# philip-bl/dctn

Measured on AMD Instinct MI355X. Metric: EPS-contraction windows/sec (fwd+bwd), higher is better.
Workload: dtype bf16; 1 GPU; cfg2 EPS[(3,4)]+linear bf16 B1024/GPU; parallelism=dp1

## Files before the change

### dctn_amd/csrc/common.h

```cpp
#pragma once
#include <hip/hip_runtime.h>
#include <stdint.h>

#include "../../include/dctn_amd.h"

typedef __bf16 bf16_t;

template <typename S> struct AccOf { typedef float type; };
template <> struct AccOf<double> { typedef double type; };

#define DCTN_WAVE 64

#ifndef DCTN_WT_FEATURES
#define DCTN_WT_FEATURES 16
#endif
#ifndef DCTN_WT_TILES
#define DCTN_WT_TILES 0
#endif

struct DctnDev { int cus; int lds; };
const DctnDev& dctn_dev();
int dctn_lds_wg_max();
long long dctn_resident_wgs(size_t lds_bytes, int lo, int hi);
bool dctn_lds_optin(const void* fn, size_t bytes);

#define DCTN_CHECK_LAUNCH()                                   \
  do {                                                        \
    if (hipGetLastError() != hipSuccess) return DCTN_ERR_LAUNCH; \
  } while (0)

void dctn_set_last_kernel(const char* name);

int dctn_zero_async(void* ptr, size_t bytes, hipStream_t st);

static inline long long ipow_ll(long long b, int e) {
  long long r = 1;
  for (int i = 0; i < e; ++i) r *= b;
  return r;
}

static inline size_t dtype_size(int dtype) {
  return dtype == DCTN_F64 ? 8 : (dtype == DCTN_F32 ? 4 : 2);
}

template <typename T>
__device__ __forceinline__ T wave_reduce_sum(T v) {
#pragma unroll
  for (int off = 32; off > 0; off >>= 1) v += __shfl_xor(v, off, 64);
  return v;
}

__device__ __forceinline__ void philox4x32_10(unsigned c0, unsigned c1, unsigned c2, unsigned c3, unsigned k0,
                                              unsigned k1, unsigned (&w)[4]) {
#pragma unroll
  for (int r = 0; r < 10; ++r) {
    const unsigned hi0 = __umulhi(0xD2511F53u, c0), lo0 = 0xD2511F53u * c0;
    const unsigned hi1 = __umulhi(0xCD9E8D57u, c2), lo1 = 0xCD9E8D57u * c2;
    c0 = hi1 ^ c1 ^ k0, c1 = lo1, c2 = hi0 ^ c3 ^ k1, c3 = lo0;
    k0 += 0x9E3779B9u, k1 += 0xBB67AE85u;
  }
  w[0] = c0, w[1] = c1, w[2] = c2, w[3] = c3;
}

struct EpsP {
  int C, B, H, W, Q, K, O, N, Ho, Wo;
  long long Wn;
  long long R;
  long long s[5];
  int m, LO, NH;
  long long HI;
  int bits;
  int opts;
};

int eps_fill_params(EpsP& p, const int64_t x_strides[5], int C, int B, int H, int W, int Q, int K,
                    int O, int policy = 0);

int eps_fwd_generic(const void* x, const void* core, void* out, void* ws, size_t ws_bytes, EpsP p, int dtype,
                    hipStream_t st);
size_t eps_bwd_generic_workspace(const EpsP& p, int dtype, int need_dx, int need_dcore);
int eps_bwd_generic(const void* x, const void* core, const void* dY, void* dX, void* dCore,
                    void* ws, size_t ws_bytes, EpsP p, int dtype, hipStream_t st);

int eps_gather_dx_launch(const void* gxw, void* dX, const EpsP& p, int dtype, hipStream_t st);

size_t eps_fwd_bigcore_workspace(const EpsP& p, int dtype, int precision);
size_t eps_bigcore_saved_bytes(const EpsP& p, int dtype, int precision);
int eps_fwd_bigcore(const void* x, const void* core, void* out, void* ws, size_t ws_bytes,
                    const EpsP& p, int dtype, int precision, hipStream_t st, void* zsave = nullptr);
size_t eps_bwd_dcore_bigcore_workspace(const EpsP& p, int dtype, int precision);
int eps_bwd_dcore_bigcore(const void* x, const void* dY, void* dCore, const EpsP& p, int dtype,
                          int precision, hipStream_t st, void* ws = nullptr, size_t ws_bytes = 0);
size_t eps_bwd_dfactor_bigcore_workspace(const EpsP& p, int dtype, int precision);
int eps_bwd_dx_bigcore(const void* x, const void* core, const void* dY, void* dX, void* ws,
                       size_t ws_bytes, const EpsP& p, int dtype, int precision, hipStream_t st,
                       const void* zsaved = nullptr, size_t zsaved_bytes = 0);

bool eps_bf16x3_covers(const EpsP& p, int dtype, int precision);
size_t eps_fwd_bf16x3_workspace(const EpsP& p, int dtype, int precision);
size_t eps_bf16x3_saved_bytes(const EpsP& p, int dtype, int precision);
int eps_fwd_bf16x3(const void* x, const void* core, void* out, void* ws, size_t ws_bytes, const EpsP& p, int dtype,
                   int precision, hipStream_t st, void* zsave = nullptr);
size_t eps_bwd_dfactor_bf16x3_workspace(const EpsP& p, int dtype, int precision);
int eps_bwd_dx_bf16x3(const void* x, const void* core, const void* dY, void* dX, void* ws, size_t ws_bytes, const EpsP& p,
                      int dtype, int precision, hipStream_t st, const void* zsaved = nullptr, size_t zsaved_bytes = 0);
size_t eps_bwd_dcore_bf16x3_workspace(const EpsP& p, int dtype, int precision);
int eps_bwd_dcore_bf16x3(const void* x, const void* dY, void* dCore, const EpsP& p, int dtype, int precision,
                         hipStream_t st, void* ws = nullptr, size_t ws_bytes = 0);

bool eps_q2f32_covers(const EpsP& p, int dtype, int precision);
int eps_fwd_q2f32(const void* x, const void* core, void* out, const EpsP& p, int dtype, int precision, hipStream_t st);
size_t eps_bwd_q2f32_workspace(const EpsP& p, int dtype, int precision);
int eps_bwd_q2f32(const void* x, const void* dY, void* dCore, void* ws, size_t ws_bytes, const EpsP& p, int dtype,
                  int precision, hipStream_t st);
int eps_head_fwd_q2f32(const void* x, const void* core, const void* head_w, const void* bias, void* feat, void* logits,
                       const EpsP& p, int Cout, int dtype, int precision, hipStream_t st);
size_t eps_head_bwd_q2f32_workspace(const EpsP& p, int Cout, int dtype, int precision);
int eps_head_bwd_q2f32(const void* x, const void* feat, const void* dLogits, const void* head_w, void* dCore, void* dW,
                       void* dBias, void* ws, size_t ws_bytes, const EpsP& p, int Cout, int dtype, int precision,
                       hipStream_t st);

bool eps_mfma_covers(const EpsP& p, int dtype, int precision);
bool eps_bigcore_covers(const EpsP& p, int dtype, int precision);

bool eps_halves_wanted(const EpsP& p, int dtype);
size_t eps_fwd_halves_workspace(const EpsP& p, int dtype);
size_t eps_halves_saved_bytes(const EpsP& p, int dtype);
int eps_fwd_halves(const void* x, const void* core, void* out, void* ws, size_t ws_bytes, const EpsP& p, int dtype,
                   hipStream_t st, void* saved = nullptr);
size_t eps_bwd_halves_workspace(const EpsP& p, int dtype, int need_dx, int need_dcore);
int eps_bwd_halves(const void* x, const void* core, const void* dY, void* dX, void* dCore, void* ws, size_t ws_bytes,
                   const EpsP& p, int dtype, hipStream_t st, const void* saved = nullptr, size_t saved_bytes = 0);

int eps_fwd_mfma(const void* x, const void* core, void* out, const EpsP& p, int dtype,
                 int precision, hipStream_t st, double* stats = nullptr);
int eps_out_stats(const void* y, long long n, int dtype, double* stats, hipStream_t st);
size_t eps_bwd_mfma_workspace(const EpsP& p, int dtype, int precision, int need_dx, int need_dcore);
int eps_bwd_mfma(const void* x, const void* core, const void* dY, void* dX, void* dCore, void* ws,
                 size_t ws_bytes, const EpsP& p, int dtype, int precision, hipStream_t st);
int eps_head_fwd_mfma(const void* x, const void* core, const void* head_w, const void* bias, void* feat, void* logits,
                      const EpsP& p, int Cout, int dtype, int precision, hipStream_t st);
size_t eps_head_bwd_mfma_workspace(const EpsP& p, int Cout, int dtype, int precision);
int eps_head_bwd_mfma(const void* x, const void* feat, const void* dLogits, const void* head_w, void* dCore,
                      void* dW, void* dBias, void* ws, size_t ws_bytes, const EpsP& p, int Cout, int dtype,
                      int precision, hipStream_t st);

struct SbsShape {
  int n;
  const int *out_sizes, *bond_sizes, *pos_h, *pos_w;
  int C, B, H, W, q, dtype;
};
static inline SbsShape sbs_string(SbsShape many, int i) {
  many.out_sizes += i * many.n;
  many.bond_sizes += i * many.n;
  many.pos_h += i * many.n;
  many.pos_w += i * many.n;
  return many;
}

size_t convsbs_saved_states_bytes(const SbsShape& sh);
int convsbs_fwd_mfma(const void* x, const int64_t xs[5], const void* const* cores, void* out, const SbsShape& sh,
                     hipStream_t st, float* save_states = nullptr);
int convsbs_bwd_mfma(const void* x, const int64_t xs[5], const void* const* cores, const void* dY, float* states, float* gxw,
                     float* const* dcores, const SbsShape& sh, hipStream_t st, float* partials = nullptr,
                     size_t partial_bytes = 0, const float* saved_states = nullptr);
bool convsbs_band_covers(const SbsShape& sh);
size_t convsbs_band_bwd_workspace(const SbsShape& sh);
int convsbs_fwd_band(const void* x, const int64_t xs[5], const void* const* cores, void* out, const SbsShape& sh,
                     hipStream_t st);
int convsbs_bwd_band(const void* x, const int64_t xs[5], const void* const* cores, const void* dY, void* dX,
// ... 22 lines not shown
```

### dctn_amd/csrc/eps_mfma.hip

```cpp
#include "common.h"

#include <cstdlib>
#include <type_traits>

typedef __attribute__((ext_vector_type(8))) __bf16 bf16x8;
typedef __attribute__((ext_vector_type(16))) float f32x16;
typedef __attribute__((ext_vector_type(8))) float f32x8;
typedef __attribute__((ext_vector_type(2))) int int2v;
typedef __attribute__((ext_vector_type(4))) int int4v;
typedef __attribute__((ext_vector_type(2))) float f32x2;

namespace {

constexpr int ilog2(int v) { return v <= 1 ? 0 : 1 + ilog2(v >> 1); }

template <typename S> __device__ __forceinline__ float to_f32(S v) { return (float)v; }

__device__ __forceinline__ float half_sum(float v) {
  const int iv = __float_as_int(v);
  const int2v r = __builtin_amdgcn_permlane32_swap(iv, iv, false, false);
  return __int_as_float(r[0]) + __int_as_float(r[1]);
}

__device__ __forceinline__ void swap_halves(float& a, float& b) {
  const int2v r = __builtin_amdgcn_permlane32_swap(__float_as_int(a), __float_as_int(b), false, false);
  a = __int_as_float(r[0]);
  b = __int_as_float(r[1]);
}
__device__ __forceinline__ void swap_halves(bf16x8& a, bf16x8& b) {
  int4v ia = __builtin_bit_cast(int4v, a), ib = __builtin_bit_cast(int4v, b);
#pragma unroll
  for (int i = 0; i < 4; ++i) {
    const int2v r = __builtin_amdgcn_permlane32_swap(ia[i], ib[i], false, false);
    ia[i] = r[0];
    ib[i] = r[1];
  }
  a = __builtin_bit_cast(bf16x8, ia);
  b = __builtin_bit_cast(bf16x8, ib);
}

__device__ __forceinline__ void wave_lds_sync() {
  __builtin_amdgcn_fence(__ATOMIC_RELEASE, "wavefront");
  __builtin_amdgcn_wave_barrier();
  __builtin_amdgcn_fence(__ATOMIC_ACQUIRE, "wavefront");
}

typedef short s16x4 __attribute__((ext_vector_type(4)));
typedef short s16x8 __attribute__((ext_vector_type(8)));
constexpr int LROW = 32;
struct TrLane {
  int wr[4];
  int rd_lo, rd_hi;
};
__device__ __forceinline__ TrLane tr_lane(int lane) {
  TrLane t;
#pragma unroll
  for (int c = 0; c < 4; ++c) t.wr[c] = lane * LROW + (((c + (lane >> 1)) & 3) << 3);
  const int g = lane >> 4, q = (lane >> 2) & 3, pp = lane & 3;
  const int lc = 2 * (g & 1) + (pp >> 1), half = pp & 1;
  const int row = 8 * (g >> 1) + q;
  t.rd_lo = row * LROW + (((lc + (row >> 1)) & 3) << 3) + 4 * half;
  t.rd_hi = (row + 4) * LROW + (((lc + ((row + 4) >> 1)) & 3) << 3) + 4 * half;
  return t;
}
__device__ __forceinline__ bf16x8 tr_frag(const short* tile, int ks, const TrLane& t) {
  typedef __attribute__((address_space(3))) s16x4 lds_s16x4;
  const s16x4 lo = __builtin_amdgcn_ds_read_tr16_b64_v4i16((lds_s16x4*)(tile + t.rd_lo + ks * 16 * LROW));
  const s16x4 hi = __builtin_amdgcn_ds_read_tr16_b64_v4i16((lds_s16x4*)(tile + t.rd_hi + ks * 16 * LROW));
  const s16x8 v = {lo[0], lo[1], lo[2], lo[3], hi[0], hi[1], hi[2], hi[3]};
  return __builtin_bit_cast(bf16x8, v);
}

struct FastDiv {
  unsigned M, s1, s2;
};
__device__ __forceinline__ unsigned fdiv(unsigned n, const FastDiv& d) {
  const unsigned t = __umulhi(d.M, n);
  return (t + ((n - t) >> d.s1)) >> d.s2;
}

#define MFMA_MAXN 16
struct MfmaP {
  int C, B, K, O, Ho, Wo;
  int P;
  int npg;
  int spc, nchunks;
  unsigned foffb[MFMA_MAXN];
  unsigned rowoffb[MFMA_MAXN];
  unsigned s1b, s2b, s3b, s4b;
  unsigned x_bytes;
  unsigned o_bytes, o_s1b;
  FastDiv div_wo;
  int rowvec_ok;
  int vec_ok;
  int Cout;
  unsigned hw_rowb, hw_bytes;
  int ncb;
  int skew;
  int opts;
#ifdef DCTN_STAMPS
  unsigned long long* stamps;
#endif
};

#ifdef DCTN_STAMPS
#define DCTN_STAMP(P, SLOT)                                                                      \
  do {                                                                                           \
    __builtin_amdgcn_sched_barrier(0);                                                           \
    unsigned long long t_;                                                                       \
    asm volatile("s_memrealtime %0\n\ts_waitcnt lgkmcnt(0)" : "=s"(t_)::"memory");               \
    if ((P).stamps && threadIdx.x == 0) (P).stamps[(long long)blockIdx.x * 8 + (SLOT)] = t_;     \
    __builtin_amdgcn_sched_barrier(0);                                                           \
  } while (0)
static unsigned long long* g_stamps = nullptr;
void dctn_stamps_set(unsigned long long* p) { g_stamps = p; }
__device__ unsigned long long* g_dev_stamps = nullptr;
void dctn_reduce_stamps_set(unsigned long long* p) { (void)hipMemcpyToSymbol(HIP_SYMBOL(g_dev_stamps), &p, sizeof(p)); }
#define DCTN_STAMP_T(P, SLOT, TID)                                                              \
  do {                                                                                           \
    __builtin_amdgcn_sched_barrier(0);                                                           \
    unsigned long long t_;                                                                       \
    asm volatile("s_memrealtime %0\n\ts_waitcnt lgkmcnt(0)" : "=s"(t_)::"memory");               \
    if ((P).stamps && threadIdx.x == (TID)) (P).stamps[(long long)blockIdx.x * 8 + (SLOT)] = t_;  \
    __builtin_amdgcn_sched_barrier(0);                                                           \
  } while (0)
#define DCTN_STAMP_ROLE_ROW 1024
#define DCTN_STAMP_R(P, SLOT)                                                                    \
  do {                                                                                           \
    __builtin_amdgcn_sched_barrier(0);                                                           \
    unsigned long long t_;                                                                       \
    asm volatile("s_memrealtime %0\n\ts_waitcnt lgkmcnt(0)" : "=s"(t_)::"memory");               \
    if ((P).stamps && threadIdx.x == 64 * 8)                                                     \
      (P).stamps[(long long)(DCTN_STAMP_ROLE_ROW + blockIdx.x) * 8 + (SLOT)] = t_;               \
    __builtin_amdgcn_sched_barrier(0);                                                           \
  } while (0)
#define DCTN_STAMP_WAVE_ROW 1536
#define DCTN_STAMP_W(P, WV)                                                                      \
  do {                                                                                           \
    __builtin_amdgcn_sched_barrier(0);                                                           \
    unsigned long long t_;                                                                       \
    asm volatile("s_memrealtime %0\n\ts_waitcnt lgkmcnt(0)" : "=s"(t_)::"memory");               \
    if ((P).stamps && (threadIdx.x & 63) == 0 && (WV) < 8)                                        \
      (P).stamps[(long long)(DCTN_STAMP_WAVE_ROW + blockIdx.x) * 8 + (WV)] = t_;                 \
    __builtin_amdgcn_sched_barrier(0);                                                           \
  } while (0)
#define DCTN_STAMP_G(SLOT)                                                                       \
  do {                                                                                           \
    __builtin_amdgcn_sched_barrier(0);                                                           \
    unsigned long long t_;                                                                       \
    asm volatile("s_memrealtime %0\n\ts_waitcnt lgkmcnt(0)" : "=s"(t_)::"memory");               \
    if (g_dev_stamps && threadIdx.x == 0) g_dev_stamps[(long long)blockIdx.x * 8 + (SLOT)] = t_;  \
    __builtin_amdgcn_sched_barrier(0);                                                           \
  } while (0)
#else
#define DCTN_STAMP(P, SLOT) do { } while (0)
#define DCTN_STAMP_T(P, SLOT, TID) do { } while (0)
#define DCTN_STAMP_G(SLOT) do { } while (0)
#define DCTN_STAMP_R(P, SLOT) do { } while (0)
#define DCTN_STAMP_W(P, WV) do { } while (0)
#endif

typedef __attribute__((ext_vector_type(4))) unsigned u32x4;
typedef __attribute__((ext_vector_type(2))) unsigned u32x2;
typedef __attribute__((ext_vector_type(2))) __bf16 bf16x2;

__device__ __forceinline__ __amdgpu_buffer_rsrc_t make_rsrc(const void* ptr, unsigned bytes) {
  return __builtin_amdgcn_make_buffer_rsrc(const_cast<void*>(ptr), 0, (int)bytes, 0x00020000);
}

template <typename S, int N, bool VEC, int ROWS>
struct RawWindow {
  u32x4 row[ROWS > 0 ? ROWS : 1];
  unsigned v[(ROWS == 0 && VEC) ? N * (int)(sizeof(S) / 2) : 1];
  unsigned e[(ROWS == 0 && !VEC) ? 2 * N : 1];
};

template <typename S, int N, bool VEC, int ROWS>
__device__ __forceinline__ void issue_window(__amdgpu_buffer_rsrc_t rs, unsigned voff, unsigned soff,
                                             const MfmaP& p, RawWindow<S, N, VEC, ROWS>& raw) {
  if constexpr (ROWS > 0) {
#pragma unroll
    for (int rw = 0; rw < ROWS; ++rw)
      raw.row[rw] = __builtin_amdgcn_raw_buffer_load_b128(rs, voff, soff + p.rowoffb[rw], 0);
  } else if constexpr (VEC) {
#pragma unroll
    for (int n = 0; n < N; ++n) {
      if constexpr (sizeof(S) == 2) {
        raw.v[n] = __builtin_amdgcn_raw_buffer_load_b32(rs, voff, soff + p.foffb[n], 0);
      } else {
        const u32x2 t = __builtin_amdgcn_raw_buffer_load_b64(rs, voff, soff + p.foffb[n], 0);
        raw.v[2 * n] = t.x;
        raw.v[2 * n + 1] = t.y;
      }
    }
  } else {
#pragma unroll
    for (int n = 0; n < N; ++n)
#pragma unroll
      for (int q = 0; q < 2; ++q) {
        if constexpr (sizeof(S) == 2)
          raw.e[2 * n + q] = (unsigned)(unsigned short)__builtin_amdgcn_raw_buffer_load_b16(
              rs, voff, soff + p.foffb[n] + q * p.s4b, 0);
        else
          raw.e[2 * n + q] = __builtin_amdgcn_raw_buffer_load_b32(rs, voff, soff + p.foffb[n] + q * p.s4b, 0);
      }
  }
}

template <typename S, int N, bool VEC, int ROWS>
__device__ __forceinline__ void unpack_window(const RawWindow<S, N, VEC, ROWS>& raw, float (&xv)[N][2]) {
  if constexpr (ROWS > 0) {
    constexpr int KK = N / ROWS;
    constexpr int CC = ROWS * ROWS / N;
#pragma unroll
    for (int rw = 0; rw < ROWS; ++rw) {
      const unsigned d[4] = {raw.row[rw].x, raw.row[rw].y, raw.row[rw].z, raw.row[rw].w};
#pragma unroll
      for (int dw = 0; dw < KK; ++dw) {
        const int n = ((rw / CC) * KK + dw) * CC + (rw % CC);
        xv[n][0] = __uint_as_float(d[dw] << 16);
        xv[n][1] = __uint_as_float(d[dw] & 0xffff0000u);
      }
    }
  } else if constexpr (VEC) {
#pragma unroll
    for (int n = 0; n < N; ++n) {
      if constexpr (sizeof(S) == 2) {
        xv[n][0] = __uint_as_float(raw.v[n] << 16);
        xv[n][1] = __uint_as_float(raw.v[n] & 0xffff0000u);
      } else {
        xv[n][0] = __uint_as_float(raw.v[2 * n]);
        xv[n][1] = __uint_as_float(raw.v[2 * n + 1]);
      }
    }
  } else {
#pragma unroll
    for (int n = 0; n < N; ++n)
#pragma unroll
      for (int q = 0; q < 2; ++q)
        xv[n][q] = sizeof(S) == 2 ? __uint_as_float(raw.e[2 * n + q] << 16) : __uint_as_float(raw.e[2 * n + q]);
  }
}

template <typename S, int OP>
struct RawRow {
  static constexpr int DW = OP * (int)sizeof(S) / 4;
  unsigned d[DW];
  unsigned e[OP];
};
template <typename S, int OP, bool VEC>
__device__ __forceinline__ void issue_row(__amdgpu_buffer_rsrc_t rs, unsigned voff, unsigned soff, int O,
                                          RawRow<S, OP>& r) {
// ... 334 lines not shown
    }
    core_commit(e0, tmp);
  }
  __syncthreads();
  bf16x8 cf[MT][KS];
#pragma unroll
  for (int t = 0; t < MT; ++t)
#pragma unroll
    for (int s = 0; s < KS; ++s)
      cf[t][s] = *reinterpret_cast<const bf16x8*>(&cs[((t * KS + s) * 64 + lane) * 8]);
#pragma unroll
  for (int u = 1; u < HEAD_FWD_HS; ++u)
    issue_window<S, N, true, ROWS>(rs_x, voff_x, (unsigned)first_of_group(u) * p.s1b, p, raw[u]);
  bf16x8 wf[HK];
  {
    const __amdgpu_buffer_rsrc_t rs_hw = make_rsrc(hw, p.hw_bytes);
    const int c = lane & 15, g = lane >> 4;
    const unsigned base = c < p.Cout ? (unsigned)c * p.hw_rowb + (unsigned)(wv * 64 * OP + 8 * g) * 2u : p.hw_bytes;
#pragma unroll
    for (int ks = 0; ks < HK; ++ks)
      wf[ks] = __builtin_bit_cast(bf16x8, __builtin_amdgcn_raw_buffer_load_b128(rs_hw, base, (unsigned)(ks * 64), 0));
  }
  __builtin_amdgcn_sched_barrier(0);

  short* tile = &ftile[wv][0];
  const int bcol = (lane & 15) < HEAD_FWD_HS ? (lane & 15) : HEAD_FWD_HS - 1;
  const short* brd = tile + bcol * SROW + 8 * (lane >> 4);
  DCTN_STAMP(p, 1);
  for (int g0 = b0, grp = 0; g0 < b1; g0 += HEAD_FWD_HS, ++grp) {
    const int g1 = g0 + HEAD_FWD_HS < b1 ? g0 + HEAD_FWD_HS : b1;
#pragma unroll
    for (int u = 0; u < HEAD_FWD_HS; ++u) {
      const int b = g0 + u;
      if (b >= g1) break;
      float xv[N][2];
      unpack_window<S, N, true, ROWS>(raw[u], xv);
      {
        const int bn = b + HEAD_FWD_HS < b1 ? b + HEAD_FWD_HS : b1 - 1;
        issue_window<S, N, true, ROWS>(rs_x, voff_x, (unsigned)bn * p.s1b, p, raw[u]);
        __builtin_amdgcn_sched_barrier(0);
      }
      bf16x8 pf0[KS], pf1[KS];
      build_p0<N0>(xv, pf0, pf1);
#pragma unroll
      for (int s = 0; s < KS; ++s) swap_halves(pf0[s], pf1[s]);
      float m0[BN / 2], m1[BN / 2];
      {
        float ph[BN / 2];
        ph[0] = xv[N - 2][0];
        ph[1] = xv[N - 2][1];
#pragma unroll
        for (int u = 2; u < N1; ++u)
#pragma unroll
          for (int bh = (1 << (u - 1)) - 1; bh >= 0; --bh) {
            const f32x2 pr = bmul2(ph[bh], f32x2{xv[N - 1 - u][0], xv[N - 1 - u][1]});
            ph[bh] = pr[0];
            ph[bh | (1 << (u - 1))] = pr[1];
          }
#pragma unroll
        for (int bh = 0; bh < BN / 2; ++bh) {
          const f32x2 mm = bmul2(ph[bh], f32x2{xv[N - 1][0], xv[N - 1][1]});
          m0[bh] = mm[0];
          m1[bh] = mm[1];
          swap_halves(m0[bh], m1[bh]);
        }
      }
      float res0[OP], res1[OP];
#pragma unroll
      for (int o = 0; o < OP; ++o) { res0[o] = 0.f; res1[o] = 0.f; }
#pragma unroll
      for (int t = 0; t < MT; ++t) {
#pragma unroll
        for (int set = 0; set < 2; ++set) {
          f32x16 acc;
#pragma unroll
          for (int v = 0; v < 16; ++v) acc[v] = 0.f;
#pragma unroll
          for (int s = 0; s < KS; ++s)
            acc = __builtin_amdgcn_mfma_f32_32x32x16_bf16(cf[t][s], set ? pf1[s] : pf0[s], acc, 0, 0, 0);
#pragma unroll
          for (int v = 0; v < 16; v += 2) {
            const int code = (t << 4) | ((v >> 2) << 2) | (v & 3);
            const float mm = set ? m1[code >> LOGO] : m0[code >> LOGO];
            float* dst = set ? res1 : res0;
            const int o = code & (OP - 1);
            const f32x2 r = bfma2(mm, f32x2{acc[v], acc[v + 1]}, f32x2{dst[o], dst[o + 1]});
            dst[o] = r[0];
            dst[o + 1] = r[1];
          }
        }
      }
      unsigned pk[OP / 2];
#pragma unroll
      for (int i = 0; i < OP / 2; ++i) {
        float a0 = res0[2 * i], a1 = res1[2 * i], c0 = res0[2 * i + 1], c1 = res1[2 * i + 1];
        swap_halves(a0, a1);
        swap_halves(c0, c1);
        pk[i] = pack_bf16(a0 + a1, c0 + c1);
      }
      if constexpr (OP == 2) {
        __builtin_amdgcn_raw_buffer_store_b32(pk[0], rs_o, voff_o, (unsigned)b * p.o_s1b, 0);
        *reinterpret_cast<unsigned*>(tile + (b - g0) * SROW + lane * OP) = pk[0];
      } else if constexpr (OP == 4) {
        __builtin_amdgcn_raw_buffer_store_b64(u32x2{pk[0], pk[1]}, rs_o, voff_o, (unsigned)b * p.o_s1b, 0);
        *reinterpret_cast<u32x2*>(tile + (b - g0) * SROW + lane * OP) = u32x2{pk[0], pk[1]};
      } else {
#pragma unroll
        for (int i = 0; i < OP / 8; ++i) {
          const u32x4 q = u32x4{pk[4 * i], pk[4 * i + 1], pk[4 * i + 2], pk[4 * i + 3]};
          __builtin_amdgcn_raw_buffer_store_b128(q, rs_o, voff_o, (unsigned)b * p.o_s1b + 16u * i, 0);
          *reinterpret_cast<u32x4*>(tile + (b - g0) * SROW + lane * OP + 8 * i) = q;
        }
      }
      if (b == b0) DCTN_STAMP(p, 2);
    }
    wave_lds_sync();
    f32x4v hd = {0.f, 0.f, 0.f, 0.f};
#pragma unroll
    for (int ks = 0; ks < HK; ++ks) {
      const bf16x8 fb = *reinterpret_cast<const bf16x8*>(brd + 32 * ks);
      hd = __builtin_amdgcn_mfma_f32_16x16x32_bf16(wf[ks], fb, hd, 0, 0, 0);
    }
    wave_lds_sync();
    {
      const int sl = lane & 15, cb = 4 * (lane >> 4);
      if (sl < g1 - g0) {
#pragma unroll
        for (int v = 0; v < 4; ++v) hsum[grp & 1][sl][cb + v][wv] = hd[v];
      }
    }
    DCTN_STAMP(p, 3);
    __syncthreads();
    for (int e = tid; e < (g1 - g0) * p.Cout; e += (int)blockDim.x) {
      const int sl = e / p.Cout, c = e - sl * p.Cout;
      float t = (float)bias[c];
      for (int w = 0; w < nwv; ++w) t += hsum[grp & 1][sl][c][w];
      logits[(long long)(g0 + sl) * p.Cout + c] = (bf16_t)t;
    }
  }
  DCTN_STAMP(p, 4);
}

constexpr int HEADT_WAVES = 16;
constexpr int HEADT_GS = 4;
constexpr int HEADT_MAXKS = 6;
constexpr int headt_pitch(int F) { return (F + 31) / 32 * 32 + 8; }

template <int N0, int N1, int OP, int ROWS, bool BLK4>
__global__ __launch_bounds__(64 * HEADT_WAVES) void eps_fwd_head_q2reg_t_k(const bf16_t* __restrict__ x,
                                                                           const bf16_t* __restrict__ core,
                                                                           const bf16_t* __restrict__ hw,
                                                                           const bf16_t* __restrict__ bias,
                                                                           bf16_t* __restrict__ out,
                                                                           bf16_t* __restrict__ logits, MfmaP p) {
  typedef bf16_t S;
  typedef __attribute__((ext_vector_type(4))) float f32x4v;
  constexpr int N = N0 + N1, A = 1 << N0, BN = 1 << N1, KS = A / 16, MT = BN * OP / 32;
  constexpr int LOGO = ilog2(OP);
  constexpr int TOT = A * BN * OP;
  static_assert(OP % 2 == 0 && TOT % 4 == 0, "outputs are handled as bf16 pairs");
  __shared__ __attribute__((aligned(16))) bf16_t cs[TOT];
  __shared__ float hsum[HEADT_WAVES][HEADT_GS][16];
  __shared__ unsigned step_ctr;
  extern __shared__ __attribute__((aligned(16))) short ftile[];
  const int tid = threadIdx.x, lane = tid & 63;
  const int wv = __builtin_amdgcn_readfirstlane(tid >> 6);
  const int b0 = (int)blockIdx.x * p.spc, b1 = b0 + p.spc < p.B ? b0 + p.spc : p.B;
  const int F = p.P * OP, LP = headt_pitch(F);
  const __amdgpu_buffer_rsrc_t rs_x = make_rsrc(x, p.x_bytes), rs_o = make_rsrc(out, p.o_bytes);
  __shared__ float bias_s[16];
  DCTN_STAMP(p, 0);
  float bias_v = 0.f;
  for (int e0 = 0; e0 < TOT; e0 += 4 * 64 * HEADT_WAVES) {
    S tmp[4];
#pragma unroll
    for (int i = 0; i < 4; ++i) {
      const int ec = e0 + tid + i * 64 * HEADT_WAVES, e = ec < TOT ? ec : TOT - 1, o = e % OP, ab = e / OP;
      tmp[i] = core[(long long)ab * p.O + (o < p.O ? o : 0)];
    }
    if (e0 == 0 && wv == 0) bias_v = (float)bias[(lane & 15) < p.Cout ? (lane & 15) : 0];
#pragma unroll
    for (int i = 0; i < 4; ++i) {
      const int e = e0 + tid + i * 64 * HEADT_WAVES, o = e % OP, ab = e / OP, bb = ab % BN, aa = ab / BN;
      const int code = ((bb >> 1) << LOGO) | o;
      const int row = (((code >> 2) & 3) << 3) | ((bb & 1) << 2) | (code & 3);
      const int dst = ((((code >> 4) * KS + (aa >> 4)) * 64 + ((aa >> 3) & 1) * 32 + row) << 3) | (aa & 7);
      if (e < TOT) cs[dst] = o < p.O ? tmp[i] : (bf16_t)0.f;
    }
  }
  if (wv == 0) bias_s[lane & 15] = bias_v;
  for (int e = tid; e < HEADT_GS * (LP - F); e += 64 * HEADT_WAVES) ftile[(e / (LP - F)) * LP + F + e % (LP - F)] = 0;
  __syncthreads();
  bf16x8 cf[MT][KS];
#pragma unroll
  for (int t = 0; t < MT; ++t)
#pragma unroll
    for (int s = 0; s < KS; ++s)
      cf[t][s] = *reinterpret_cast<const bf16x8*>(&cs[((t * KS + s) * 64 + lane) * 8]);
  DCTN_STAMP(p, 1);

  auto lane_at = [&](int pg, bool live, unsigned& voff_x, unsigned& voff_o, int& pos) {
    pos = pg * 64 + lane;
    const bool valid = live && pos < p.P;
    const unsigned pu = (unsigned)(pos < p.P ? pos : p.P - 1);
    const unsigned ho = fdiv(pu, p.div_wo), wo = pu - ho * (unsigned)p.Wo;
    voff_x = valid ? ho * p.s2b + wo * p.s3b : p.x_bytes;
    voff_o = valid ? pu * (unsigned)(OP * 2) : p.o_bytes;
  };
  auto draw = [&]() {
    unsigned v = 0;
    if (lane == 0) v = __hip_atomic_fetch_add(&step_ctr, 1u, __ATOMIC_RELAXED, __HIP_MEMORY_SCOPE_WORKGROUP);
    return (int)__builtin_amdgcn_readfirstlane(v);
  };

  for (int g0 = b0; g0 < b1; g0 += HEADT_GS) {
    const int ng = g0 + HEADT_GS < b1 ? HEADT_GS : b1 - g0;
    const int nsteps = ng * p.npg;
    if (tid == 0) step_ctr = 2 * HEADT_WAVES;
    __syncthreads();
    int cur = wv, nxt = wv + HEADT_WAVES;
    int s = cur / p.npg, pg = cur - s * p.npg, pos;
    unsigned voff_x, voff_o;
    lane_at(pg, cur < nsteps, voff_x, voff_o, pos);
    RawWindow<S, N, true, ROWS> raw;
    issue_window<S, N, true, ROWS>(rs_x, voff_x, (unsigned)(g0 + (cur < nsteps ? s : 0)) * p.s1b, p, raw);
#ifdef DCTN_STAMPS
    bool first_step = true;
#endif
    while (cur < nsteps) {
      float xv[N][2];
      unpack_window<S, N, true, ROWS>(raw, xv);
      const unsigned vo = voff_o, so = (unsigned)(g0 + s) * p.o_s1b;
      short* trow = ftile + s * LP + (pos < p.P ? pos : 0) * OP;
      const bool tvalid = pos < p.P;
      {
        cur = nxt;
        s = cur / p.npg;
        pg = cur - s * p.npg;
        lane_at(pg, cur < nsteps, voff_x, voff_o, pos);
        issue_window<S, N, true, ROWS>(rs_x, voff_x, (unsigned)(g0 + (cur < nsteps ? s : 0)) * p.s1b, p, raw);
        nxt = draw();
        __builtin_amdgcn_sched_barrier(0);
      }
      bf16x8 pf0[KS], pf1[KS];
      build_p0<N0>(xv, pf0, pf1);
#pragma unroll
      for (int s2 = 0; s2 < KS; ++s2) swap_halves(pf0[s2], pf1[s2]);
      float m0[BN / 2], m1[BN / 2];
      {
        float ph[BN / 2];
        ph[0] = xv[N - 2][0];
        ph[1] = xv[N - 2][1];
#pragma unroll
        for (int u = 2; u < N1; ++u)
#pragma unroll
          for (int bh = (1 << (u - 1)) - 1; bh >= 0; --bh) {
            const f32x2 pr = bmul2(ph[bh], f32x2{xv[N - 1 - u][0], xv[N - 1 - u][1]});
            ph[bh] = pr[0];
            ph[bh | (1 << (u - 1))] = pr[1];
          }
#pragma unroll
        for (int bh = 0; bh < BN / 2; ++bh) {
          const f32x2 mm = bmul2(ph[bh], f32x2{xv[N - 1][0], xv[N - 1][1]});
          m0[bh] = mm[0];
          m1[bh] = mm[1];
          swap_halves(m0[bh], m1[bh]);
        }
      }
      float res0[OP], res1[OP];
#pragma unroll
      for (int o = 0; o < OP; ++o) { res0[o] = 0.f; res1[o] = 0.f; }
#pragma unroll
      for (int t = 0; t < MT; ++t) {
#pragma unroll
        for (int set = 0; set < 2; ++set) {
          f32x16 acc;
#pragma unroll
          for (int v = 0; v < 16; ++v) acc[v] = 0.f;
#pragma unroll
          for (int s2 = 0; s2 < KS; ++s2)
            acc = __builtin_amdgcn_mfma_f32_32x32x16_bf16(cf[t][s2], set ? pf1[s2] : pf0[s2], acc, 0, 0, 0);
#pragma unroll
          for (int v = 0; v < 16; v += 2) {
            const int code = (t << 4) | ((v >> 2) << 2) | (v & 3);
            const float mm = set ? m1[code >> LOGO] : m0[code >> LOGO];
            float* dst = set ? res1 : res0;
            const int o = code & (OP - 1);
            const f32x2 r = __builtin_elementwise_fma(f32x2{mm, mm}, f32x2{acc[v], acc[v + 1]}, f32x2{dst[o], dst[o + 1]});
            dst[o] = r[0];
            dst[o + 1] = r[1];
          }
        }
      }
      unsigned pk[OP / 2];
#pragma unroll
      for (int i = 0; i < OP / 2; ++i) {
        float a0 = res0[2 * i], a1 = res1[2 * i], c0 = res0[2 * i + 1], c1 = res1[2 * i + 1];
        swap_halves(a0, a1);
        swap_halves(c0, c1);
        pk[i] = pack_bf16(a0 + a1, c0 + c1);
      }
      if constexpr (OP == 2) {
        if constexpr (!BLK4) __builtin_amdgcn_raw_buffer_store_b32(pk[0], rs_o, vo, so, 0);
        if (tvalid) *reinterpret_cast<unsigned*>(trow) = pk[0];
      } else if constexpr (OP == 4) {
        if constexpr (!BLK4) __builtin_amdgcn_raw_buffer_store_b64(u32x2{pk[0], pk[1]}, rs_o, vo, so, 0);
        if (tvalid) *reinterpret_cast<u32x2*>(trow) = u32x2{pk[0], pk[1]};
      } else {
#pragma unroll
        for (int i = 0; i < OP / 8; ++i) {
          const u32x4 q = u32x4{pk[4 * i], pk[4 * i + 1], pk[4 * i + 2], pk[4 * i + 3]};
          if constexpr (!BLK4) __builtin_amdgcn_raw_buffer_store_b128(q, rs_o, vo, so + 16u * i, 0);
          if (tvalid) *reinterpret_cast<u32x4*>(trow + 8 * i) = q;
        }
      }
#ifdef DCTN_STAMPS
      if (first_step) DCTN_STAMP(p, 2);
      first_step = false;
#endif
    }
    DCTN_STAMP(p, 3);
    DCTN_STAMP_T(p, 4, 64 * (HEADT_WAVES - 1));
    const int nks = (F + 31) / 32;
    const int c = lane & 15, kg = lane >> 4;
    const __amdgpu_buffer_rsrc_t rs_hw = make_rsrc(hw, p.hw_bytes);
    u32x4 wf[HEADT_MAXKS];
#pragma unroll
    for (int i = 0; i < HEADT_MAXKS; ++i) {
      const int ks = wv + HEADT_WAVES * i, k = 32 * ks + 8 * kg;
      const unsigned vo2 = (ks < nks && c < p.Cout && k + 7 < F) ? (unsigned)c * p.hw_rowb + (unsigned)k * 2u : p.hw_bytes;
      wf[i] = __builtin_amdgcn_raw_buffer_load_b128(rs_hw, vo2, 0, 0);
    }
    __syncthreads();
    DCTN_STAMP(p, 5);
    if constexpr (BLK4) {
      static_assert(HEADT_GS == 4, "a group is one block of the blocked4 layout");
      const unsigned sob = (unsigned)(g0 >> 2) * (unsigned)F * 8u;
      for (int f = 2 * tid; f < F; f += 2 * 64 * HEADT_WAVES) {
        unsigned r[HEADT_GS];
#pragma unroll
        for (int i = 0; i < HEADT_GS; ++i) r[i] = i < ng ? *reinterpret_cast<const unsigned*>(ftile + i * LP + f) : 0u;
        const u32x4 q = u32x4{__builtin_amdgcn_perm(r[1], r[0], 0x05040100u), __builtin_amdgcn_perm(r[3], r[2], 0x05040100u),
                              __builtin_amdgcn_perm(r[1], r[0], 0x07060302u), __builtin_amdgcn_perm(r[3], r[2], 0x07060302u)};
        __builtin_amdgcn_raw_buffer_store_b128(q, rs_o, (unsigned)f * 8u, sob, DCTN_WT_FEATURES);
      }
    }
    __builtin_amdgcn_sched_barrier(0);
    f32x4v hd = {0.f, 0.f, 0.f, 0.f};
    const short* brd = ftile + (c < HEADT_GS ? c : HEADT_GS - 1) * LP + 8 * kg;
#pragma unroll
    for (int i = 0; i < HEADT_MAXKS; ++i) {
      const int ks = wv + HEADT_WAVES * i;
      if (ks < nks) {
        const bf16x8 fb = *reinterpret_cast<const bf16x8*>(brd + 32 * ks);
        hd = __builtin_amdgcn_mfma_f32_16x16x32_bf16(__builtin_bit_cast(bf16x8, wf[i]), fb, hd, 0, 0, 0);
      }
    }
    if (c < HEADT_GS) {
#pragma unroll
      for (int v = 0; v < 4; ++v) hsum[wv][c][4 * kg + v] = hd[v];
    }
    __syncthreads();
    if (tid < HEADT_GS * 16) {
      const int sl = tid >> 4, cc = tid & 15;
      if (sl < ng && cc < p.Cout) {
        float t = bias_s[cc];
#pragma unroll
        for (int w = 0; w < HEADT_WAVES; ++w) t += hsum[w][sl][cc];
        logits[(long long)(g0 + sl) * p.Cout + cc] = (bf16_t)t;
      }
    }
  }
  DCTN_STAMP(p, 6);
}

constexpr int BWD_WAVES = 8;
constexpr size_t dcore_dyn_lds_bytes(int mt) { return (size_t)BWD_WAVES * (1 + mt) * 64 * 32 * sizeof(short); }

__device__ __forceinline__ void head_dw_role_waves(const bf16_t* __restrict__ feat, const bf16_t* __restrict__ dL,
                                                   bf16_t* __restrict__ dW, int B, int Cout, long long F, int n_dw,
                                                   int rw, float* __restrict__ lds, const MfmaP& p);
template <typename S, int N0, int N1, int OP, bool XVEC, bool OVEC, int ROWS, int HEADC, int DWROLE = 0>
__global__ __launch_bounds__(64 * (BWD_WAVES + DWROLE)) void eps_bwd_dcore_q2reg_k(const S* __restrict__ x,
                                                             const S* __restrict__ dY,
                                                             const S* __restrict__ hw,
                                                             const S* __restrict__ feat,
                                                             float* __restrict__ partial,
                                                             float* __restrict__ dwpart, MfmaP p,
                                                             S* __restrict__ dW, int n_dw) {
  constexpr int N = N0 + N1, A = 1 << N0, BN = 1 << N1, KS = A / 16, MT = BN * OP / 32;
  constexpr int AT = A >= 32 ? A / 32 : 1;
  constexpr int LOGO = ilog2(OP);
  constexpr bool LDST = A == 32 && MT <= 2;
// ... 686 lines not shown
                                                          bf16_t* __restrict__ dW, int ncb, long long nW, int n_dw,
                                                          const bf16_t* __restrict__ dL,
                                                          bf16_t* __restrict__ dBias, int B, int Cout,
                                                          const bf16_t* __restrict__ feat, int gemm) {
  __shared__ float red[32][33];
  const int tid = threadIdx.x;
  const int bid = gemm == 2 && (int)blockIdx.x < n_core + n_dw
                      ? ((int)blockIdx.x < n_dw ? n_core + (int)blockIdx.x : (int)blockIdx.x - n_dw)
                      : (int)blockIdx.x;
  if (bid < n_core) {
    DCTN_STAMP_G(0);
    const int c = tid & 31, k32 = tid >> 5;
    const long long stride = (long long)BN * OP * ACOLS;
    const long long e = (long long)bid * 32 + c;
    float acc = 0.f;
    for (int k0 = 0; k0 < nblk; k0 += 256) {
      float v[8];
#pragma unroll
      for (int i = 0; i < 8; ++i) {
        const int k = k0 + k32 + 32 * i;
        const float ld = partial[(k < nblk ? k : nblk - 1) * stride + e];
        v[i] = k < nblk ? ld : 0.f;
      }
      acc += ((v[0] + v[1]) + (v[2] + v[3])) + ((v[4] + v[5]) + (v[6] + v[7]));
    }
    red[k32][c] = acc;
    __syncthreads();
    if (k32 == 0) {
      float t = 0.f;
#pragma unroll
      for (int i = 0; i < 32; ++i) t += red[i][c];
      const int m = (int)(e / ACOLS), a = (int)(e % ACOLS);
      const int b = m / OP, o = m % OP;
      if (a < A && o < O) dCore[((long long)a * BN + b) * O + o] = (bf16_t)t;
    }
    DCTN_STAMP_G(4);
    return;
  }
  if (bid < n_core + n_dw) {
    if (!dW) return;
    if (gemm) {
      extern __shared__ __attribute__((aligned(16))) float gemm_lds[];
      if (gemm == 2) head_dw_gemm_role<DWG_BFW, true>(feat, dL, dW, B, Cout, nW / Cout, bid - n_core, gemm_lds);
      else head_dw_gemm_role<DWG_FW, false>(feat, dL, dW, B, Cout, nW / Cout, bid - n_core, gemm_lds);
      return;
    }
    const long long e = (long long)(bid - n_core) * 256 + (tid >> 2);
    const int sub = tid & 3;
    float v[8];
#pragma unroll
    for (int i = 0; i < 8; ++i) {
      const int k = sub + 4 * i;
      const float ld = dwpart[(long long)(k < ncb ? k : ncb - 1) * nW + (e < nW ? e : nW - 1)];
      v[i] = (k < ncb && e < nW) ? ld : 0.f;
    }
    float t = ((v[0] + v[1]) + (v[2] + v[3])) + ((v[4] + v[5]) + (v[6] + v[7]));
    for (int k = 32 + sub; k < ncb; k += 4) t += e < nW ? dwpart[(long long)k * nW + e] : 0.f;
    t += __shfl_xor(t, 1, 64);
    t += __shfl_xor(t, 2, 64);
    if (sub == 0 && e < nW) dW[e] = (bf16_t)t;
    return;
  }
  if (!dBias) return;
  {
    const int c = tid & 15, j = tid >> 4;
    float t = 0.f;
    if (c < Cout) {
      int b = j;
      for (; b + 64 * 7 < B; b += 64 * 8) {
        float v[8];
#pragma unroll
        for (int i = 0; i < 8; ++i) v[i] = (float)dL[(long long)(b + 64 * i) * Cout + c];
        t += ((v[0] + v[1]) + (v[2] + v[3])) + ((v[4] + v[5]) + (v[6] + v[7]));
      }
      for (; b < B; b += 64) t += (float)dL[(long long)b * Cout + c];
    }
    __shared__ float rb[64][17];
    rb[j][c] = t;
    __syncthreads();
    if (tid < 16 && tid < Cout) {
      float u = 0.f;
#pragma unroll 8
      for (int i = 0; i < 64; ++i) u += rb[i][tid];
      dBias[tid] = (bf16_t)u;
    }
  }
}

int next_pow2(int v) {
  int r = 1;
  while (r < v) r <<= 1;
  return r;
}

bool family_ok(const EpsP& p, int dtype, int precision) {
  if (p.Q != 2) return false;
  if (dtype == DCTN_F64) return false;
  if (dtype == DCTN_F32 && precision != DCTN_PREC_BF16) return false;
  if (p.N != 8 && p.N != 9) return false;
  const long long esz = dtype == DCTN_BF16 ? 2 : 4;
  {
    long long ext = 0;
    const long long dims[5] = {p.C, p.B, p.H, p.W, p.Q};
    for (int i = 0; i < 5; ++i) {
      if (p.s[i] < 0) return false;
      ext += (dims[i] - 1) * p.s[i];
    }
    if ((ext + 1) * esz >= (1LL << 31)) return false;
    if (p.Wn * p.O * esz >= (1LL << 31)) return false;
  }
  const int op = next_pow2(p.O);
  return op >= 2 ? op <= 16 : true;
}

FastDiv make_fastdiv(unsigned d) {
  FastDiv f;
  if (d <= 1) {
    f.M = 0; f.s1 = 0; f.s2 = 0;
    return f;
  }
  unsigned l = 0;
  while ((1ull << l) < d) ++l;
  f.M = (unsigned)(((1ull << 32) * ((1ull << l) - d)) / d + 1);
  f.s1 = 1;
  f.s2 = l - 1;
  return f;
}

void fill_mp(MfmaP& m, const EpsP& p, const void* x, int dtype) {
  const long long esz = dtype == DCTN_BF16 ? 2 : 4;
  for (int n = 0; n < p.N && n < MFMA_MAXN; ++n) {
    const int pos = n / p.C, ch = n - pos * p.C;
    const int dh = pos / p.K, dw = pos - dh * p.K;
    m.foffb[n] = (unsigned)((ch * p.s[0] + dh * p.s[2] + dw * p.s[3]) * esz);
  }
  m.s1b = (unsigned)(p.s[1] * esz); m.s2b = (unsigned)(p.s[2] * esz);
  m.s3b = (unsigned)(p.s[3] * esz); m.s4b = (unsigned)(p.s[4] * esz);
  long long ext = 0;
  const long long dims[5] = {p.C, p.B, p.H, p.W, p.Q};
  for (int i = 0; i < 5; ++i) ext += (dims[i] - 1) * p.s[i];
  m.x_bytes = (unsigned)((ext + 1) * esz);
  const int rows = p.K * p.C;
  for (int rw = 0; rw < MFMA_MAXN; ++rw) m.rowoffb[rw] = 0;
  for (int rw = 0; rw < rows && rw < MFMA_MAXN; ++rw) {
    const int dh = rw / p.C, ch = rw - dh * p.C;
    m.rowoffb[rw] = (unsigned)((ch * p.s[0] + dh * p.s[2]) * esz);
  }
  m.rowvec_ok = dtype == DCTN_BF16 && p.s[4] == 1 && p.s[3] == 2 && p.K <= 4 && rows <= MFMA_MAXN / 2 &&
                ((p.N == 9 && rows == 3) || (p.N == 8 && rows == 4));
  m.div_wo = make_fastdiv((unsigned)p.Wo);
  m.C = p.C; m.B = p.B; m.K = p.K; m.O = p.O; m.Ho = p.Ho; m.Wo = p.Wo;
  m.P = p.Ho * p.Wo;
  m.npg = (m.P + 63) / 64;
  m.spc = 1; m.nchunks = p.B;
  m.o_s1b = (unsigned)((long long)m.P * p.O * esz);
  m.o_bytes = (unsigned)(p.Wn * p.O * esz);
  m.vec_ok = p.s[4] == 1 && p.s[0] % 2 == 0 && p.s[1] % 2 == 0 && p.s[2] % 2 == 0 &&
             p.s[3] % 2 == 0 && ((uintptr_t)x % 4) == 0;
  m.Cout = 0; m.hw_rowb = 0; m.hw_bytes = 0; m.ncb = 0; m.skew = 0;
  m.opts = p.opts;
#ifdef DCTN_STAMPS
  m.stamps = g_stamps;
#endif
}

constexpr int FWD_BLOCKS_PER_CU = 4;

template <int N0, int N1, int OP>
constexpr size_t dcore_dyn_lds() {
  constexpr int A = 1 << N0, MT = (1 << N1) * OP / 32;
  return (A == 32 && MT <= 2) ? (size_t)BWD_WAVES * (1 + MT) * 64 * LROW * sizeof(short) : 0;
}
#define DCTN_DCORE_LAUNCH(KERNEL, G, B, DYN, ST, ...)                                                  \
  do {                                                                                                 \
    if ((DYN) > 0 && !dctn_lds_optin((const void*)KERNEL, DYN)) return DCTN_ERR_UNSUPPORTED;       \
    hipLaunchKernelGGL(KERNEL, G, B, DYN, ST, __VA_ARGS__);                                            \
  } while (0)

int plan_waves(MfmaP& m, int wpb, long long target) {
  long long chunks = target / m.npg;
  if (chunks < 1) chunks = 1;
  if (chunks > m.B) chunks = m.B;
  m.spc = (int)((m.B + chunks - 1) / chunks);
  m.nchunks = (m.B + m.spc - 1) / m.spc;
  const long long waves = (long long)m.nchunks * m.npg;
  long long blocks = (waves + wpb - 1) / wpb;
  if (blocks >= 8) blocks = (blocks + 7) / 8 * 8;
  return (int)blocks;
}

template <typename S>
bool row_vec_ok(const MfmaP& m, int OP, const void* ptr) {
  return m.O == OP && ((uintptr_t)ptr % 4) == 0 && (OP * sizeof(S)) % 4 == 0;
}

template <typename S, int N0, int N1, int OP>
int fwd_launch_t(const void* x, const void* core, void* out, double* stats, const MfmaP& m_in, hipStream_t st) {
  MfmaP m = m_in;
  const int blocks = plan_waves(m, 4, (long long)FWD_BLOCKS_PER_CU * dctn_dev().cus * 4);
  const bool ovec = out == nullptr || row_vec_ok<S>(m, OP, out);
  const dim3 g((unsigned)blocks), b(256);
  constexpr int NN = N0 + N1;
  constexpr int RW = NN == 9 ? 3 : 4;
  if (m.rowvec_ok && m.vec_ok && ovec && sizeof(S) == 2)
    hipLaunchKernelGGL((eps_fwd_q2reg_k<S, N0, N1, OP, true, true, RW>), g, b, 0, st, (const S*)x,
                       (const S*)core, (S*)out, stats, m);
  else if (m.vec_ok && ovec)
    hipLaunchKernelGGL((eps_fwd_q2reg_k<S, N0, N1, OP, true, true, 0>), g, b, 0, st, (const S*)x,
                       (const S*)core, (S*)out, stats, m);
  else if (m.vec_ok)
    hipLaunchKernelGGL((eps_fwd_q2reg_k<S, N0, N1, OP, true, false, 0>), g, b, 0, st, (const S*)x,
                       (const S*)core, (S*)out, stats, m);
  else
    hipLaunchKernelGGL((eps_fwd_q2reg_k<S, N0, N1, OP, false, false, 0>), g, b, 0, st, (const S*)x,
                       (const S*)core, (S*)out, stats, m);
  DCTN_CHECK_LAUNCH();
  dctn_set_last_kernel("eps_fwd_mfma_q2reg");
  return DCTN_OK;
}

template <typename S, int N0, int N1, int OP>
int bwd_launch_t(const void* x, const void* dY, void* dCore, void* ws, const MfmaP& m_in,
                 hipStream_t st) {
  constexpr int A = 1 << N0, BN = 1 << N1, AT = A >= 32 ? A / 32 : 1;
  constexpr size_t DYN = dcore_dyn_lds<N0, N1, OP>();
  MfmaP m = m_in;
  const int grid = plan_waves(m, BWD_WAVES, (long long)dctn_dev().cus * BWD_WAVES);
  const bool ovec = row_vec_ok<S>(m, OP, dY);
  const dim3 g(grid), b(64 * BWD_WAVES);
  constexpr int NN = N0 + N1;
  constexpr int RW = NN == 9 ? 3 : 4;
  if (m.rowvec_ok && m.vec_ok && ovec && sizeof(S) == 2)
    DCTN_DCORE_LAUNCH((eps_bwd_dcore_q2reg_k<S, N0, N1, OP, true, true, RW, 0>), g, b, DYN, st,
                       (const S*)x, (const S*)dY, (const S*)nullptr, (const S*)nullptr, (float*)ws, (float*)nullptr, m, (S*)nullptr, 0);
  else if (m.vec_ok && ovec)
    DCTN_DCORE_LAUNCH((eps_bwd_dcore_q2reg_k<S, N0, N1, OP, true, true, 0, 0>), g, b, DYN, st,
                       (const S*)x, (const S*)dY, (const S*)nullptr, (const S*)nullptr, (float*)ws, (float*)nullptr, m, (S*)nullptr, 0);
  else if (m.vec_ok)
    DCTN_DCORE_LAUNCH((eps_bwd_dcore_q2reg_k<S, N0, N1, OP, true, false, 0, 0>), g, b, DYN, st,
                       (const S*)x, (const S*)dY, (const S*)nullptr, (const S*)nullptr, (float*)ws, (float*)nullptr, m, (S*)nullptr, 0);
  else
    DCTN_DCORE_LAUNCH((eps_bwd_dcore_q2reg_k<S, N0, N1, OP, false, false, 0, 0>), g, b, DYN, st,
                       (const S*)x, (const S*)dY, (const S*)nullptr, (const S*)nullptr, (float*)ws, (float*)nullptr, m, (S*)nullptr, 0);
  DCTN_CHECK_LAUNCH();
  if (m.opts & DCTN_OPT_MAIN_KERNEL_ONLY) return DCTN_PARTIAL;
  hipLaunchKernelGGL((eps_bwd_dcore_reduce_k<S>), dim3(BN * OP * AT), dim3(256), 0, st,
                     (const float*)ws, (S*)dCore, grid, A, BN, m.O, OP, AT * 32);
  DCTN_CHECK_LAUNCH();
  dctn_set_last_kernel("eps_bwd_mfma_q2reg");
  return DCTN_OK;
}

#ifndef DCTN_DCORE_SKEW
#define DCTN_DCORE_SKEW(spc) ((spc) / 3)
#endif

int plan_grouped(MfmaP& m) {
  if (m.npg > dctn_dev().cus) return 0;
  long long ncb = dctn_dev().cus / m.npg;
  const long long need = (m.B + BWD_WAVES - 1) / BWD_WAVES;
  if (ncb > need) ncb = need;
  m.spc = (int)((m.B + ncb * BWD_WAVES - 1) / (ncb * BWD_WAVES));
  m.nchunks = (m.B + m.spc - 1) / m.spc;
  m.ncb = (m.nchunks + BWD_WAVES - 1) / BWD_WAVES;
  long long blocks = (long long)m.ncb * m.npg;
  if (blocks >= 8) blocks = (blocks + 7) / 8 * 8;
  return blocks <= dctn_dev().cus ? (int)blocks : 0;
}

size_t head_dw_partial_bytes(const EpsP& p, int Cout) {
  const long long P = (long long)p.Ho * p.Wo, npg = (P + 63) / 64;
  if (npg > dctn_dev().cus) return 0;
  return (size_t)(dctn_dev().cus / npg) * ((size_t)Cout * (size_t)(P * p.O) + 16) * sizeof(float);
}

long long blocked4_bytes(const MfmaP& m) { return (long long)(m.B + 3) / 4 * 4 * m.P * m.O * 2; }
template <int N0, int N1, int OP>
bool head_blocked4_ok(const MfmaP& m) {
  constexpr int A = 1 << N0, MT = (1 << N1) * OP / 32;
  const long long F = (long long)m.P * OP;
  return A == 32 && MT <= 2 && OP == 4 && m.vec_ok && blocked4_bytes(m) < (1LL << 31) && !(m.opts & DCTN_OPT_SMALL_CHUNKS) &&
         F % 8 == 0 && F <= (long long)HEADT_WAVES * HEADT_MAXKS * 32;
}

template <int N0, int N1, int OP>
int bwd_head_launch_t(const void* x, const void* dL, const void* hw, const void* feat, void* dCore, void* dW,
                      void* dBias, void* ws, size_t core_ws_bytes, const MfmaP& m_in, hipStream_t st) {
  typedef bf16_t S;
  constexpr int A = 1 << N0, BN = 1 << N1, AT = A >= 32 ? A / 32 : 1;
  constexpr size_t DYN = dcore_dyn_lds<N0, N1, OP>();
  MfmaP m = m_in;
  const bool blk = (m.opts & DCTN_OPT_HEAD_FEATURES_BLOCKED4) != 0;
  if (m.O != OP || m.Cout < 2 || m.Cout > 16 || m.Cout % 2 != 0) return DCTN_ERR_UNSUPPORTED;
  if (((uintptr_t)dL % 4) != 0 || ((uintptr_t)hw % 4) != 0 || ((uintptr_t)feat % (blk ? 16 : 4)) != 0) return DCTN_ERR_UNSUPPORTED;
  if (blk && !head_blocked4_ok<N0, N1, OP>(m)) return DCTN_ERR_UNSUPPORTED;
  const int grid = plan_grouped(m);
  if (grid == 0) return DCTN_ERR_UNSUPPORTED;
  float* dwpart = reinterpret_cast<float*>(static_cast<unsigned char*>(ws) + core_ws_bytes);
  const long long nW = (long long)m.Cout * m.P * OP;
  constexpr int MT = BN * OP / 32;
  const bool headmm = A == 32 && MT <= 2 && OP == 4 && m.vec_ok;
  if (headmm && (long long)m.B * m.P * OP * 2 >= (1LL << 31)) return DCTN_ERR_UNSUPPORTED;
  const bool gemm = headmm;
  m.skew = headmm ? DCTN_DCORE_SKEW(m.spc) : 0;
  if (m.skew >= m.spc) m.skew = m.spc - 1;

// ... 216 lines not shown
```

Before: 28.05 billion windows/s.

## Issue first window load during core staging and tabulate per-position offsets in LDS

```diff
diff --git a/dctn_amd/csrc/common.h b/dctn_amd/csrc/common.h
--- a/dctn_amd/csrc/common.h
+++ b/dctn_amd/csrc/common.h
@@ -16,6 +16,16 @@
 #endif
 #ifndef DCTN_WT_TILES
 #define DCTN_WT_TILES 0
+#endif
+
+#ifndef DCTN_FWD_ARGS_ONCE
+#define DCTN_FWD_ARGS_ONCE 0
+#endif
+#ifndef DCTN_FWD_EARLY_WINDOW
+#define DCTN_FWD_EARLY_WINDOW 1
+#endif
+#ifndef DCTN_FWD_POS_TABLE
+#define DCTN_FWD_POS_TABLE 1
 #endif
 
 struct DctnDev { int cus; int lds; };
diff --git a/dctn_amd/csrc/eps_mfma.hip b/dctn_amd/csrc/eps_mfma.hip
--- a/dctn_amd/csrc/eps_mfma.hip
+++ b/dctn_amd/csrc/eps_mfma.hip
@@ -98,6 +98,7 @@
   int ncb;
   int skew;
   int opts;
+  unsigned npg_rcp;
 #ifdef DCTN_STAMPS
   unsigned long long* stamps;
 #endif
@@ -738,16 +739,30 @@
                                                                            const bf16_t* __restrict__ hw,
                                                                            const bf16_t* __restrict__ bias,
                                                                            bf16_t* __restrict__ out,
-                                                                           bf16_t* __restrict__ logits, MfmaP p) {
+                                                                           bf16_t* __restrict__ logits, MfmaP p_in) {
   typedef bf16_t S;
   typedef __attribute__((ext_vector_type(4))) float f32x4v;
   constexpr int N = N0 + N1, A = 1 << N0, BN = 1 << N1, KS = A / 16, MT = BN * OP / 32;
   constexpr int LOGO = ilog2(OP);
   constexpr int TOT = A * BN * OP;
   static_assert(OP % 2 == 0 && TOT % 4 == 0, "outputs are handled as bf16 pairs");
+#if DCTN_FWD_ARGS_ONCE
+  MfmaP p = p_in;
+  asm volatile("" ::"s"(x), "s"(core), "s"(hw), "s"(bias), "s"(out), "s"(logits), "s"(p.B), "s"(p.O), "s"(p.Wo), "s"(p.P),
+               "s"(p.npg), "s"(p.spc), "s"(p.rowoffb[0]), "s"(p.rowoffb[1]), "s"(p.rowoffb[2]), "s"(p.rowoffb[ROWS - 1]),
+               "s"(p.s1b), "s"(p.s2b), "s"(p.s3b), "s"(p.x_bytes), "s"(p.o_bytes), "s"(p.o_s1b), "s"(p.div_wo.M),
+               "s"(p.div_wo.s1), "s"(p.div_wo.s2), "s"(p.Cout), "s"(p.hw_rowb), "s"(p.hw_bytes), "s"(p.npg_rcp));
+#else
+  const MfmaP& p = p_in;
+#endif
   __shared__ __attribute__((aligned(16))) bf16_t cs[TOT];
   __shared__ float hsum[HEADT_WAVES][HEADT_GS][16];
   __shared__ unsigned step_ctr;
+#if DCTN_FWD_POS_TABLE
+  static_assert((HEAD_FWD_MAXPG + 1) * 64 <= 64 * HEADT_WAVES, "one table entry per thread");
+  __shared__ u32x2 pos_tab[(HEAD_FWD_MAXPG + 1) * 64];
+#endif
+  constexpr unsigned POS_NONE = 0x80000000u;
   extern __shared__ __attribute__((aligned(16))) short ftile[];
   const int tid = threadIdx.x, lane = tid & 63;
   const int wv = __builtin_amdgcn_readfirstlane(tid >> 6);
@@ -757,6 +772,26 @@
   __shared__ float bias_s[16];
   DCTN_STAMP(p, 0);
   float bias_v = 0.f;
+  auto lane_at = [&](int pos, unsigned& voff_x, unsigned& toff) {
+    const bool valid = pos < p.P;
+    const unsigned pu = (unsigned)(valid ? pos : p.P - 1);
+    const unsigned ho = fdiv(pu, p.div_wo), wo = pu - ho * (unsigned)p.Wo;
+    voff_x = valid ? ho * p.s2b + wo * p.s3b : p.x_bytes;
+    toff = valid ? pu * (unsigned)(OP * 2) : POS_NONE;
+  };
+  auto first_ticket = [&](int nsteps, int& s, unsigned& voff_x, unsigned& toff) {
+    const int sq = (int)(((unsigned)wv * p.npg_rcp) >> 16), pg = wv - sq * p.npg;
+    const bool live = wv < nsteps;
+    s = live ? sq : 0;
+    lane_at(live ? pg * 64 + lane : p.P, voff_x, toff);
+  };
+  const int ng0 = b0 + HEADT_GS < b1 ? HEADT_GS : b1 - b0, nsteps0 = ng0 * p.npg;
+  int s;
+  unsigned voff_x, toff;
+  RawWindow<S, N, true, ROWS> raw;
+#if DCTN_FWD_EARLY_WINDOW
+  if (tid == 0) step_ctr = 2 * HEADT_WAVES;
+#endif
   for (int e0 = 0; e0 < TOT; e0 += 4 * 64 * HEADT_WAVES) {
     S tmp[4];
 #pragma unroll
@@ -765,6 +800,19 @@
       tmp[i] = core[(long long)ab * p.O + (o < p.O ? o : 0)];
     }
     if (e0 == 0 && wv == 0) bias_v = (float)bias[(lane & 15) < p.Cout ? (lane & 15) : 0];
+#if DCTN_FWD_EARLY_WINDOW
+    if (e0 == 0) {
+      first_ticket(nsteps0, s, voff_x, toff);
+      issue_window<S, N, true, ROWS>(rs_x, voff_x, (unsigned)(b0 + s) * p.s1b, p, raw);
+    }
+#endif
+#if DCTN_FWD_POS_TABLE
+    if (e0 == 0 && tid < (p.npg + 1) * 64) {
+      unsigned vx, t;
+      lane_at(tid, vx, t);
+      pos_tab[tid] = u32x2{vx, t};
+    }
+#endif
 #pragma unroll
     for (int i = 0; i < 4; ++i) {
       const int e = e0 + tid + i * 64 * HEADT_WAVES, o = e % OP, ab = e / OP, bb = ab % BN, aa = ab / BN;
@@ -785,14 +833,6 @@
       cf[t][s] = *reinterpret_cast<const bf16x8*>(&cs[((t * KS + s) * 64 + lane) * 8]);
   DCTN_STAMP(p, 1);
 
-  auto lane_at = [&](int pg, bool live, unsigned& voff_x, unsigned& voff_o, int& pos) {
-    pos = pg * 64 + lane;
-    const bool valid = live && pos < p.P;
-    const unsigned pu = (unsigned)(pos < p.P ? pos : p.P - 1);
-    const unsigned ho = fdiv(pu, p.div_wo), wo = pu - ho * (unsigned)p.Wo;
-    voff_x = valid ? ho * p.s2b + wo * p.s3b : p.x_bytes;
-    voff_o = valid ? pu * (unsigned)(OP * 2) : p.o_bytes;
-  };
   auto draw = [&]() {
     unsigned v = 0;
     if (lane == 0) v = __hip_atomic_fetch_add(&step_ctr, 1u, __ATOMIC_RELAXED, __HIP_MEMORY_SCOPE_WORKGROUP);
@@ -802,29 +842,40 @@
   for (int g0 = b0; g0 < b1; g0 += HEADT_GS) {
     const int ng = g0 + HEADT_GS < b1 ? HEADT_GS : b1 - g0;
     const int nsteps = ng * p.npg;
-    if (tid == 0) step_ctr = 2 * HEADT_WAVES;
-    __syncthreads();
+    auto locate = [&](int ticket, int& s, unsigned& voff_x, unsigned& toff) {
+      const bool live = ticket < nsteps;
+#if DCTN_FWD_POS_TABLE
+      const int sq = (int)(((unsigned)ticket * p.npg_rcp) >> 16), pg = ticket - sq * p.npg;
+      s = live ? sq : 0;
+      const u32x2 e = pos_tab[(live ? pg : p.npg) * 64 + lane];
+      voff_x = e.x;
+      toff = e.y;
+#else
+      const int sq = ticket / p.npg, pg = ticket - sq * p.npg;
+      s = live ? sq : 0;
+      lane_at(live ? pg * 64 + lane : p.P, voff_x, toff);
+#endif
+    };
+    if (!DCTN_FWD_EARLY_WINDOW || g0 != b0) {
+      if (tid == 0) step_ctr = 2 * HEADT_WAVES;
+      __syncthreads();
+      first_ticket(nsteps, s, voff_x, toff);
+      issue_window<S, N, true, ROWS>(rs_x, voff_x, (unsigned)(g0 + s) * p.s1b, p, raw);
+    }
     int cur = wv, nxt = wv + HEADT_WAVES;
-    int s = cur / p.npg, pg = cur - s * p.npg, pos;
-    unsigned voff_x, voff_o;
-    lane_at(pg, cur < nsteps, voff_x, voff_o, pos);
-    RawWindow<S, N, true, ROWS> raw;
-    issue_window<S, N, true, ROWS>(rs_x, voff_x, (unsigned)(g0 + (cur < nsteps ? s : 0)) * p.s1b, p, raw);
 #ifdef DCTN_STAMPS
     bool first_step = true;
 #endif
     while (cur < nsteps) {
       float xv[N][2];
       unpack_window<S, N, true, ROWS>(raw, xv);
-      const unsigned vo = voff_o, so = (unsigned)(g0 + s) * p.o_s1b;
-      short* trow = ftile + s * LP + (pos < p.P ? pos : 0) * OP;
-      const bool tvalid = pos < p.P;
+      const unsigned vo = toff, so = (unsigned)(g0 + s) * p.o_s1b;
+      const bool tvalid = toff != POS_NONE;
+      short* trow = reinterpret_cast<short*>(reinterpret_cast<char*>(ftile + s * LP) + toff);
       {
         cur = nxt;
-        s = cur / p.npg;
-        pg = cur - s * p.npg;
-        lane_at(pg, cur < nsteps, voff_x, voff_o, pos);
-        issue_window<S, N, true, ROWS>(rs_x, voff_x, (unsigned)(g0 + (cur < nsteps ? s : 0)) * p.s1b, p, raw);
+        locate(cur, s, voff_x, toff);
+        issue_window<S, N, true, ROWS>(rs_x, voff_x, (unsigned)(g0 + s) * p.s1b, p, raw);
         nxt = draw();
         __builtin_amdgcn_sched_barrier(0);
       }
@@ -1817,6 +1868,7 @@
   m.C = p.C; m.B = p.B; m.K = p.K; m.O = p.O; m.Ho = p.Ho; m.Wo = p.Wo;
   m.P = p.Ho * p.Wo;
   m.npg = (m.P + 63) / 64;
+  m.npg_rcp = (65536u + (unsigned)m.npg - 1u) / (unsigned)m.npg;
   m.spc = 1; m.nchunks = p.B;
   m.o_s1b = (unsigned)((long long)m.P * p.O * esz);
   m.o_bytes = (unsigned)(p.Wn * p.O * esz);
```

Measured after the change: 28.60 billion windows/s (median of 6 runs). 2.0% higher.
